# jgiovatto/srsLTE

Measured on AMD Instinct MI355X. Metric: turbo decoded Mbit/s (LTE 20 MHz, K=6144, 8 half-iterations) incl. OFDM demod of the same subframes, higher is better.
Workload: dtype int16

## Files before the change

srslte_amd/csrc/turbo_kernels.hip:

```cpp
#include <type_traits>

#include "hip_common.h"
#include "turbo_arith.h"
#include "turbo_device.h"
#include "turbo_extract.h"
#include "turbo_layout.h"

namespace phyhip {
namespace turbo {

template <class AR>
__device__ __forceinline__ void beta_step(s2 (&o)[8], s2 x, s2 y)
{
  auto adds = [](s2 a, s2 b) { return AR::add_raw(a, b); };
  s2   xy   = AR::add(x, y);
  s2 n0 = vmax(adds(o[4], xy), o[0]);
  s2 n1 = vmax(o[4], adds(o[0], xy));
  s2 n2 = vmax(adds(o[5], y), adds(o[1], x));
  s2 n3 = vmax(adds(o[5], x), adds(o[1], y));
  s2 n4 = vmax(adds(o[6], x), adds(o[2], y));
  s2 n5 = vmax(adds(o[6], y), adds(o[2], x));
  s2 n6 = vmax(o[7], adds(o[3], xy));
  s2 n7 = vmax(adds(o[7], xy), o[3]);
  o[0] = AR::clean(n0);
  o[1] = AR::clean(n1);
  o[2] = AR::clean(n2);
  o[3] = AR::clean(n3);
  o[4] = AR::clean(n4);
  o[5] = AR::clean(n5);
  o[6] = AR::clean(n6);
  o[7] = AR::clean(n7);
}

template <class AR, bool WITH_LLR>
__device__ __forceinline__ s2 alpha_step(s2 (&o)[8], const s2 (&b)[8], s2 x, s2 y)
{
  auto adds = [](s2 a, s2 b) { return AR::add_raw(a, b); };
  s2   xy   = AR::add(x, y);
  s2 m_b[8], nw[8];
  m_b[0] = o[0];
  m_b[1] = adds(o[3], y);
  m_b[2] = adds(o[4], y);
  m_b[3] = o[7];
  m_b[4] = o[1];
  m_b[5] = adds(o[2], y);
  m_b[6] = adds(o[5], y);
  m_b[7] = o[6];
  nw[0] = adds(o[1], xy);
  nw[1] = adds(o[2], x);
  nw[2] = adds(o[5], x);
  nw[3] = adds(o[6], xy);
  nw[4] = adds(o[0], xy);
  nw[5] = adds(o[3], x);
  nw[6] = adds(o[4], x);
  nw[7] = adds(o[7], xy);
  s2 out = splat(0);
  if (WITH_LLR) {
    s2 m0 = adds(b[0], m_b[0]);
    s2 m1 = adds(b[0], nw[0]);
#pragma unroll
    for (int i = 1; i < 8; i++) {
      m0 = vmax(m0, adds(b[i], m_b[i]));
      m1 = vmax(m1, adds(b[i], nw[i]));
    }
    out = AR::llr(AR::clean(m1), AR::clean(m0));
  }
#pragma unroll
  for (int i = 0; i < 8; i++) {
    o[i] = AR::clean(vmax(m_b[i], nw[i]));
  }
  return out;
}

__device__ __forceinline__ void keep_ops(uint4 (&Bl)[8][2][64], uint32_t s, int lane, const s2 (&xs)[8], const s2 (&ys)[8])
{
  Bl[2 * s][0][lane]     = make_uint4(to_u(xs[0]), to_u(xs[1]), to_u(xs[2]), to_u(xs[3]));
  Bl[2 * s][1][lane]     = make_uint4(to_u(xs[4]), to_u(xs[5]), to_u(xs[6]), to_u(xs[7]));
  Bl[2 * s + 1][0][lane] = make_uint4(to_u(ys[0]), to_u(ys[1]), to_u(ys[2]), to_u(ys[3]));
  Bl[2 * s + 1][1][lane] = make_uint4(to_u(ys[4]), to_u(ys[5]), to_u(ys[6]), to_u(ys[7]));
}
__device__ __forceinline__ void kept_ops(const uint4 (&Bl)[8][2][64], uint32_t s, int lane, s2 (&xs)[8], s2 (&ys)[8])
{
  const uint4 x0 = Bl[2 * s][0][lane], x1 = Bl[2 * s][1][lane], y0 = Bl[2 * s + 1][0][lane], y1 = Bl[2 * s + 1][1][lane];
  xs[0] = from_u(x0.x), xs[1] = from_u(x0.y), xs[2] = from_u(x0.z), xs[3] = from_u(x0.w);
  xs[4] = from_u(x1.x), xs[5] = from_u(x1.y), xs[6] = from_u(x1.z), xs[7] = from_u(x1.w);
  ys[0] = from_u(y0.x), ys[1] = from_u(y0.y), ys[2] = from_u(y0.z), ys[3] = from_u(y0.w);
  ys[4] = from_u(y1.x), ys[5] = from_u(y1.y), ys[6] = from_u(y1.z), ys[7] = from_u(y1.w);
}

__device__ __forceinline__ uint32_t norm_mask(bool on)
{
  uint32_t m = __builtin_amdgcn_readfirstlane(on ? ~0u : 0u);
  asm("" : "+s"(m));
  return m;
}

template <bool WHOLE, int POS>
struct FwdBody {
  static constexpr bool value = WHOLE;
  static constexpr int  pos   = POS;
};


template <int LPC, class AR, bool ES, int CKS>
__device__ __forceinline__ void tdec_win_unit(const WinParams& p, const uint32_t wb, const int lane, uint4 (&Bl)[8][2][64],
                                              uint32_t (&Tr)[512])
{
  const uint32_t crc_poly = ES ? p.crc_poly : 0u;
  const CbDesc*  desc     = ES ? p.desc : nullptr;
  constexpr int  NB  = 2 * LPC;
  constexpr int  CPW = 64 / LPC;
  constexpr bool NT  = !ES && !AR::kIs8;
  static_assert(CKS == 8 || CKS == 16, "check-points every 8 or every 16 steps");
  static_assert(CKS == 8 || !AR::kIs8, "the 16-step form's whole-block bodies use Ar16's masked normalisation");
  using ARW = std::conditional_t<CKS == 16, AR, Ar16>;
  const int     pl   = lane % LPC;
  const uint32_t xbase = xch_group_base<LPC>(lane);
  const int     cb_raw = (int)wb * CPW + lane / LPC;
  const bool    live = cb_raw < p.n_cb;
  const int     cb   = live ? cb_raw : p.n_cb - 1;
  const uint32_t K       = p.K;
  const uint32_t long_sb = K / NB;
  const uint32_t nblk    = (long_sb + 7) >> 3;
  const uint32_t AW      = nblk * LPC * 8;

  const uint32_t AWG = AW * CPW;
  uint32_t* ws  = p.ws + (size_t)wb * p.ws_stride * CPW;
  uint32_t* S   = ws;
  uint32_t* P0  = ws + AWG;
  uint32_t* P1  = ws + 2 * AWG;
  uint32_t* A1  = ws + 3 * AWG;
  uint32_t* D   = ws + 4 * AWG;
  uint32_t* A2  = ws + 5 * AWG;
  uint32_t* CK  = ws + 6 * AWG;
  short*    TL  = reinterpret_cast<short*>(CK + (size_t)(nblk + 1) * 64 * 8) + 16 * (lane / LPC);

  if (p.n_begin == 0) {
    const bool fast = !desc && !p.in_is8 && !p.sb_layout && (long_sb & 3u) == 0 && ((reinterpret_cast<uintptr_t>(p.input) | (2u * p.in_stride)) & 7u) == 0;
    if (fast) {
      const int first = (int)wb * CPW;
      extract_input_natural16<LPC, AR>(p.input + (size_t)first * p.in_stride, p.in_stride, p.n_cb - first, K, long_sb, nblk, lane,
                                       S, P0, P1, TL - 16 * (lane / LPC), reinterpret_cast<uint2*>(&Bl[0][0][0]));
    } else if (!p.in_is8 && p.sb_layout &&
               __all(((reinterpret_cast<uintptr_t>(p.input) + 2 * (desc ? (size_t)desc[cb].in_off : (size_t)cb * p.in_stride)) & 15u) == 0)) {
      const short* in = p.input + (desc ? (size_t)desc[cb].in_off : (size_t)cb * p.in_stride);
      extract_input_sb16<LPC, AR>(in, K, long_sb >> 3, lane, pl, S, P0, P1, TL, Tr);
      if (long_sb & 7u) {
        extract_input<LPC, AR>(in, 1, K, long_sb, nblk, lane, pl, S, P0, P1, TL, long_sb >> 3, false);
      }
    } else if (p.in_is8) {
      const signed char* in = reinterpret_cast<const signed char*>(p.input) + (desc ? (size_t)desc[cb].in_off : (size_t)cb * p.in_stride);
      extract_input<LPC, AR>(in, p.sb_layout, K, long_sb, nblk, lane, pl, S, P0, P1, TL);
    } else {
      const short* in = p.input + (desc ? (size_t)desc[cb].in_off : (size_t)cb * p.in_stride);
      extract_input<LPC, AR>(in, p.sb_layout, K, long_sb, nblk, lane, pl, S, P0, P1, TL);
    }
  }
  const uint32_t wrap_row = (AR::kIs8 && (K & 31u)) ? long_sb - 1 : 0xffffffffu;
  __syncthreads();

  uint8_t*       out       = p.output + (desc ? (size_t)desc[cb].out_off : (size_t)cb * p.out_stride);
  const uint32_t out_bytes = desc ? desc[cb].out_bytes : K / 8;
  uint32_t m_own_v = ~0u, m_row_v = ~0u;
  auto     set_masks = [&](bool dead) {
    const unsigned long long dm = __ballot(dead);
    const int                og = AR::kIs8 ? ((8 * (lane & 7)) / LPC) * LPC : ((4 * (lane & 15)) / LPC) * LPC;
    m_own_v                     = dead ? 0u : ~0u;
    m_row_v                     = ((dm >> og) & 1ull) ? 0u : ~0u;
  };
  if (ES) {
    set_masks(!live);
  }
  auto m_own = [&]() -> uint32_t { return ES ? m_own_v : ~0u; };
  auto m_row = [&]() -> uint32_t { return ES ? m_row_v : ~0u; };
  const bool bit_rows = !ES && p.final_run && !p.dec_llr && p.n_end > p.n_begin;
  auto decide = [&](bool write, bool final_try) -> uint32_t {
    short*         o16   = (p.dec_llr && live && write) ? p.dec_llr + (size_t)cb * K : nullptr;
    const bool     whole = (long_sb & 7) == 0;
    const uint32_t bps   = long_sb >> 3;
    const uint32_t poly  = crc_poly & 0xffffffu;
    uint32_t       c0 = 0, c1 = 0;
    const uint32_t sbs  = nblk + 1;
    uint8_t*       sbuf = reinterpret_cast<uint8_t*>(&Bl[0][0][0]) + (size_t)(lane / LPC) * NB * sbs;
    static_assert(sizeof(Bl) >= 64 / LPC * 2 * LPC * (6144 / (2 * LPC) / 8 + 2), "byte image does not fit");
    if (!whole) {
      sbuf[(2 * pl) * sbs + nblk]     = 0;
      sbuf[(2 * pl + 1) * sbs + nblk] = 0;
    }
    uint4* img = &Bl[0][0][0] + (whole ? 0u : (CPW * NB * sbs + 15u) / 16u);
    if (bit_rows) {
      for (uint32_t k = lane; k < long_sb; k += 64) {
        img[k] = ws_load16<NT>(D + (size_t)k * 4);
      }
      __syncthreads();
    }
    {
      const bool wide = whole && ((bps & 3) == 0) && ((reinterpret_cast<uintptr_t>(out) & 3) == 0) && out_bytes == K / 8;
      uint32_t   w0 = 0, w1 = 0;
      uint32_t   t[8], tn[8];
      if (!bit_rows) {
        issue_rows_raw<AR::kIs8, NT>(D, 0, lane, t);
      }
      for (uint32_t b = 0; b < nblk; b++) {
        if (!bit_rows && b + 1 < nblk) {
          issue_rows_raw<AR::kIs8, NT>(D, (b + 1) & m_row(), lane, tn);
        }
        uint32_t r[8];
        if (bit_rows) {
#pragma unroll
          for (int j = 0; j < 8; j++) {
            const uint32_t k = b * 8 + j < long_sb ? b * 8 + j : long_sb - 1;
            const uint4    m = img[k];
            r[j] = (uint32_t)(((((uint64_t)m.y << 32) | m.x) >> lane) & 1u) | ((uint32_t)(((((uint64_t)m.w << 32) | m.z) >> lane) & 1u) << 16);
          }
        } else {
          rows_to_lane_v<AR::kIs8>(Tr, lane, t, r);
        }
        uint32_t b0 = 0, b1 = 0;
#pragma unroll
        for (int j = 0; j < 8; j++) {
          if (b * 8 + j < long_sb) {
            const s2       v  = from_u(r[j]);
            const uint32_t x0 = v.x > 0 ? 1u : 0u, x1 = v.y > 0 ? 1u : 0u;
            b0 |= (x0 << 7) >> j;
            b1 |= (x1 << 7) >> j;
            if (crc_poly) {
              c0 = ((c0 << 1) & 0xffffffu) ^ ((((c0 >> 23) ^ x0) & 1u) ? poly : 0u);
              c1 = ((c1 << 1) & 0xffffffu) ^ ((((c1 >> 23) ^ x1) & 1u) ? poly : 0u);
            }
            if (o16 && whole) {
              o16[(2 * pl) * long_sb + b * 8 + j]     = AR::out16(v.x);
              o16[(2 * pl + 1) * long_sb + b * 8 + j] = AR::out16(v.y);
            }
          }
        }
        if (!whole) {
          sbuf[(2 * pl) * sbs + b]     = (uint8_t)b0;
          sbuf[(2 * pl + 1) * sbs + b] = (uint8_t)b1;
        }
        if (whole && write && live) {
          if (wide) {
            w0 |= b0 << (8 * (b & 3));
            w1 |= b1 << (8 * (b & 3));
            if ((b & 3) == 3) {
              *reinterpret_cast<uint32_t*>(out + (2 * pl) * bps + (b & ~3u))     = w0;
              *reinterpret_cast<uint32_t*>(out + (2 * pl + 1) * bps + (b & ~3u)) = w1;
              w0 = w1 = 0;
            }
          } else {
            if ((2 * pl) * bps + b < out_bytes) {
              out[(2 * pl) * bps + b] = (uint8_t)b0;
            }
            if ((2 * pl + 1) * bps + b < out_bytes) {
              out[(2 * pl + 1) * bps + b] = (uint8_t)b1;
            }
          }
        }
        if (!bit_rows) {
#pragma unroll
          for (int j = 0; j < 8; j++) {
            t[j] = tn[j];
          }
        }
      }
    }
    uint32_t crc = 0;
    if (crc_poly) {
      auto mulmod = [&](uint32_t a, uint32_t m) {
        uint32_t r = 0;
#pragma unroll 4
        for (int i = 23; i >= 0; i--) {
          r = ((r << 1) & 0xffffffu) ^ (((r >> 23) & 1u) ? poly : 0u);
          r ^= ((m >> i) & 1u) ? a : 0u;
        }
        return r;
      };
      crc = mulmod(c0, p.crc_mult[2 * pl]) ^ mulmod(c1, p.crc_mult[2 * pl + 1]);
#pragma unroll
      for (int off = LPC / 2; off > 0; off >>= 1) {
        crc ^= __shfl_xor(crc, off, LPC);
      }
    }
    __syncthreads();
    if (!whole && write && (!crc_poly || crc == 0 || final_try)) {
      const uint32_t nbytes = K / 8;
      const uint32_t lim    = out_bytes < nbytes ? out_bytes : nbytes;
      const bool     al     = (reinterpret_cast<uintptr_t>(out) & 3) == 0;
      for (uint32_t w = pl; w * 4 < nbytes; w += LPC) {
        uint32_t d = (w * 32) / long_sb, k = w * 32 - d * long_sb;
        uint32_t word = 0;
#pragma unroll
        for (int t = 0; t < 4; t++) {
          if (w * 4 + t < nbytes) {
            const uint8_t* q = sbuf + d * sbs + (k >> 3);
            uint32_t       v = ((((uint32_t)q[0] << 8) | q[1]) >> (8 - (k & 7))) & 0xffu;
            if (k + 8 > long_sb && d + 1 < (uint32_t)NB) {
              v |= (uint32_t)sbuf[(d + 1) * sbs] >> (long_sb - k);
            }
            word |= v << (8 * t);
          }
          k += 8;
          if (k >= long_sb) {
            k -= long_sb;
            d++;
          }
        }
        if (live) {
          if (al && w * 4 + 3 < lim) {
            *reinterpret_cast<uint32_t*>(out + 4 * w) = word;
          } else {
#pragma unroll
            for (int t = 0; t < 4; t++) {
              if (w * 4 + t < lim) {
                out[w * 4 + t] = (uint8_t)(word >> (8 * t));
              }
            }
          }
        }
      }
      if (o16) {
        const short* sd = reinterpret_cast<const short*>(D);
        for (uint32_t nn = pl; nn < K; nn += LPC) {
          const uint32_t d = nn / long_sb, k = nn % long_sb;
          const uint32_t e = (k * 64 + (lane / LPC) * LPC + (d >> 1)) * 2 + (d & 1);
          o16[nn] = AR::kIs8 ? (short)reinterpret_cast<const signed char*>(D)[e] : sd[e];
        }
      }
    }
    __syncthreads();
    return crc;
  };
  bool     done = false;
  uint32_t noi  = 0;

  for (uint32_t n = p.n_begin; n < p.n_end; n++) {
    const bool      dec1    = !(n & 1);
    const bool      has_app = dec1 && n > 0;
    const uint32_t* Y       = dec1 ? P0 : P1;
    const short*    xt      = dec1 ? TL : TL + 6;
    const short*    yt      = dec1 ? TL + 3 : TL + 9;

    struct Ops {
      uint32_t x[8], y[8], a[8];
    };
    constexpr std::integral_constant<bool, NT>    kStream{};
    constexpr std::integral_constant<bool, false> kReuse{};
    const uint32_t* X = dec1 ? S : A2;
    auto issue = [&](auto nt, uint32_t b, Ops& q, bool ok = true) {
      if constexpr (CKS == 16) {
        static_assert(!ES, "the early-stop masks differ between blocked and row arrays");
        const bool oka = ok && has_app;
        uint32_t   bb = ok ? b : 0u, ba = oka ? b : 0u;
        int        ln = ok ? lane : 0, la = oka ? lane : 0;
        asm volatile("" : "+v"(ln), "+v"(la));
        issue_rows_raw<AR::kIs8, nt.value>(X, bb, ln, q.x);
        issue_rows_raw<AR::kIs8, nt.value>(Y, bb, ln, q.y);
        issue_rows_raw<AR::kIs8, nt.value>(A1, ba, la, q.a);
      } else {
        if (dec1) {
          load_block_raw<AR::kIs8, NT>(S, (b & m_own()) * 64 + lane, q.x);
        } else {
          issue_rows_raw<AR::kIs8, NT>(A2, b & m_row(), lane, q.x);
        }
        load_block_raw<AR::kIs8, NT>(Y, (b & m_own()) * 64 + lane, q.y);
        if (has_app) {
          issue_rows_raw<AR::kIs8, NT>(A1, b & m_row(), lane, q.a);
        }
      }
    };
    auto prep = [&](const Ops& q, s2(&xs)[8], s2(&ys)[8], s2(&ap)[8]) {
      uint32_t xr[8], ar[8], yr[8];
      if (dec1) {
        block_values<AR::kIs8>(q.x, xr);
      } else {
        rows_to_lane_v<AR::kIs8>(Tr, lane, q.x, xr);
      }
      if (has_app) {
        rows_to_lane_v<AR::kIs8>(Tr, lane, q.a, ar);
      }
      block_values<AR::kIs8>(q.y, yr);
#pragma unroll
      for (int j = 0; j < 8; j++) {
        xs[j] = from_u(xr[j]);
        ys[j] = from_u(yr[j]);
        ap[j] = splat(0);
        if (has_app) {
          ap[j] = from_u(ar[j]);
          xs[j] = AR::add(ap[j], xs[j]);
        }
      }
    };
    auto taken = [&](const Ops& q) {
      asm volatile("" ::"v"(q.x[0]), "v"(q.x[1]), "v"(q.x[2]), "v"(q.x[3]), "v"(q.x[4]), "v"(q.x[5]), "v"(q.x[6]), "v"(q.x[7]));
      asm volatile("" ::"v"(q.y[0]), "v"(q.y[1]), "v"(q.y[2]), "v"(q.y[3]), "v"(q.y[4]), "v"(q.y[5]), "v"(q.y[6]), "v"(q.y[7]));
      if (has_app || CKS == 16) {
        asm volatile("" ::"v"(q.a[0]), "v"(q.a[1]), "v"(q.a[2]), "v"(q.a[3]), "v"(q.a[4]), "v"(q.a[5]), "v"(q.a[6]), "v"(q.a[7]));
      }
    };
    Ops cur, nxt, nx2, nx3;

    s2 fw[8];
#pragma unroll
    for (int i = 0; i < 8; i++) {
      fw[i] = splat(-AR::kInf);
    }
    {
      const uint32_t w0 = long_sb - TD_WIN_OVERLAP;
      const uint32_t bl = nblk - 1;
      issue(kStream, w0 >> 3, cur);
      for (uint32_t b = w0 >> 3; b <= bl; b++) {
        issue(kStream, b < bl ? b + 1 : TD_WIN_OVERLAP / 8 - 1, nxt);
        s2 xs[8], ys[8], ap[8];
        prep(cur, xs, ys, ap);
        if (b + 4 > bl) {
          keep_ops(Bl, b + 3 - bl, lane, xs, ys);
        }
#pragma unroll
        for (int j = 0; j < 8; j++) {
          uint32_t k = b * 8 + j;
          if (k >= w0 && k < long_sb) {
            alpha_step<AR, false>(fw, fw, xs[j], ys[j]);
            uint32_t kk = k - w0;
            if (AR::norm_at(kk)) {
              AR::normalize(fw);
            }
          }
        }
        cur = nxt;
      }
    }
#pragma unroll
    for (int i = 0; i < 8; i++) {
      uint32_t u   = to_u(fw[i]);
      uint32_t prv = __shfl_up(u, 1, LPC);
      uint32_t lo  = (pl == 0) ? (uint32_t)(uint16_t)(short)(i ? -AR::kInf : 0) : (prv >> 16);
      uint32_t hi  = u & 0xffffu;
      fw[i]        = from_u(lo | (hi << 16));
    }

    s2 o[8];
#pragma unroll
    for (int i = 0; i < 8; i++) {
      o[i] = splat(-AR::kInf);
    }
    for (int b = TD_WIN_OVERLAP / 8 - 1; b >= 0; b--) {
      if (b > 0) {
        issue(kStream, b - 1, nxt);
      }
      s2 xs[8], ys[8], ap[8];
      prep(cur, xs, ys, ap);
#pragma unroll
      for (int j = 7; j >= 0; j--) {
        beta_step<AR>(o, xs[j], ys[j]);
        uint32_t k = b * 8 + j;
        if (AR::norm_at(k)) {
          AR::normalize(o);
        }
      }
      cur = nxt;
    }
    {
      short tr[8];
      tail_trellis<AR>(xt, yt, tr);
#pragma unroll
      for (int i = 0; i < 8; i++) {
        uint32_t u   = to_u(o[i]);
        uint32_t nbr = __shfl_down(u, 1, LPC);
        uint32_t lo  = u >> 16;
        uint32_t hi  = (pl == LPC - 1) ? (uint32_t)(uint16_t)tr[i] : (nbr & 0xffffu);
        o[i]         = from_u(lo | (hi << 16));
      }
      uint32_t ck[8];
#pragma unroll
      for (int i = 0; i < 8; i++) {
        ck[i] = to_u(o[i]);
      }
      store_block_v<AR::kIs8>(CK, (nblk & m_own()) * 64 + lane, ck);
    }
    if constexpr (CKS == 16) {
      const int top = (int)nblk - 5;
      auto      block = [&](int b, const Ops& c, Ops& tgt) {
        s2 xs[8], ys[8], ap[8];
        if (b > top) {
          kept_ops(Bl, (uint32_t)(b < (int)nblk ? b : (int)nblk - 1) + 4 - nblk, lane, xs, ys);
        } else {
          taken(c);
          prep(c, xs, ys, ap);
        }
        issue(kStream, b - 3, tgt, b >= 3 && b - 3 <= top);
        if (b < (int)nblk) {
#pragma unroll
          for (int j = 7; j >= 0; j--) {
            uint32_t k = b * 8 + j;
            if (k < long_sb) {
              beta_step<AR>(o, xs[j], ys[j]);
              if (j == 0 && b > 0 && !(b & 1)) {
                uint32_t ck[8];
#pragma unroll
                for (int i = 0; i < 8; i++) {
                  ck[i] = to_u(o[i]);
                }
                store_block_v<AR::kIs8>(CK, ((uint32_t)b & m_own()) * 64 + lane, ck);
              }
              if (AR::norm_at(k)) {
                AR::normalize(o);
              }
            }
          }
        }
      };
      auto whole_block = [&](auto nt, auto ck_store, auto bottom, int b, const Ops& c, Ops& tgt) {
        s2 xs[8], ys[8], ap[8];
        taken(c);
        prep(c, xs, ys, ap);
        issue(nt, b - 3, tgt, b >= 3);
#pragma unroll
        for (int j = 7; j >= 0; j--) {
          beta_step<AR>(o, xs[j], ys[j]);
          if constexpr (ck_store.value) {
            if (j == 0) {
              uint32_t ck[8];
#pragma unroll
              for (int i = 0; i < 8; i++) {
                ck[i] = to_u(o[i]);
              }
              store_block_v<AR::kIs8>(CK, ((uint32_t)b & m_own()) * 64 + lane, ck);
            }
          }
          if (bottom.value && j == 0) {
            AR::normalize_if(o, norm_mask(b != 0));
          } else if (AR::norm_in_block(j)) {
            AR::normalize(o);
          }
        }
      };
      constexpr std::integral_constant<bool, true>  kStore{}, kBottom{};
      constexpr std::integral_constant<bool, false> kNoStore{}, kInner{};
      int b = ((int)nblk - 1) | 3;
#pragma nounroll
      for (; b > top; b -= 4) {
        block(b, nx3, cur);
        block(b - 1, nx2, nx3);
        block(b - 2, nxt, nx2);
        block(b - 3, cur, nxt);
      }
      const int b_reuse = p.reuse_blocks ? (int)p.reuse_blocks + 6 : 3;
#pragma nounroll
      for (; b >= b_reuse; b -= 4) {
        whole_block(kStream, kNoStore, kInner, b, nx3, cur);
        whole_block(kStream, kStore, kInner, b - 1, nx2, nx3);
        whole_block(kStream, kNoStore, kInner, b - 2, nxt, nx2);
        whole_block(kStream, kStore, kBottom, b - 3, cur, nxt);
      }
#pragma nounroll
      for (; b >= 3; b -= 4) {
        whole_block(kReuse, kNoStore, kInner, b, nx3, cur);
        whole_block(kReuse, kStore, kInner, b - 1, nx2, nx3);
        whole_block(kReuse, kNoStore, kInner, b - 2, nxt, nx2);
        whole_block(kReuse, kStore, kBottom, b - 3, cur, nxt);
      }
    } else {
      for (int b = (int)nblk - 1; b >= 0; b--) {
        const bool ahead = b + 3 <= (int)nblk;
        if (b > 1 && ahead) {
          issue(kStream, b - 2, nx2);
        }
        s2 xs[8], ys[8], ap[8];
        if (b + 4 >= (int)nblk) {
          kept_ops(Bl, (uint32_t)b + 4 - nblk, lane, xs, ys);
        } else {
          prep(cur, xs, ys, ap);
        }
#pragma unroll
        for (int j = 7; j >= 0; j--) {
          uint32_t k = b * 8 + j;
          if (k < long_sb) {
            beta_step<AR>(o, xs[j], ys[j]);
            if (j == 0 && b > 0 && (CKS == 8 || !(b & 1))) {
              uint32_t ck[8];
#pragma unroll
              for (int i = 0; i < 8; i++) {
                ck[i] = to_u(o[i]);
              }
              store_block_v<AR::kIs8>(CK, ((uint32_t)b & m_own()) * 64 + lane, ck);
            }
            if (AR::norm_at(k)) {
              AR::normalize(o);
            }
          }
        }
        if (b > 0 && ahead) {
          cur = nxt;
          nxt = nx2;
        }
      }
    }
    __syncthreads();

#pragma unroll
    for (int i = 0; i < 8; i++) {
      o[i] = fw[i];
    }

    const uint32_t* lut = dec1 ? p.deint : p.inter;
    uint32_t*       dst = dec1 ? A2 : A1;
    const bool fuse = dec1 && n >= 2;
    uint32_t sub_x = dec1 ? 0u : ~0u;
    asm volatile("" : "+s"(sub_x));
    const bool last = (n + 1 == p.n_end) || crc_poly;
    const bool sign_rows = bit_rows && n + 1 == p.n_end;

    constexpr FwdBody<false, -1> kGeneral{};
    constexpr FwdBody<true, 0>   kWhole0{};
    constexpr FwdBody<true, 1>   kWhole1{};
    constexpr FwdBody<true, 2>   kWhole2{};
    constexpr FwdBody<true, 3>   kWhole3{};
    auto rederive_start = [&](int len, const uint32_t(&ckv)[8], s2(&st)[8]) {
#pragma unroll
      for (int i = 0; i < 8; i++) {
        st[i] = from_u(ckv[i]);
      }
      const int top = CKS == 16 ? (len - 1) & 7 : len - 1;
      Bl[top][0][lane] = make_uint4(ckv[0], ckv[1], ckv[2], ckv[3]);
      Bl[top][1][lane] = make_uint4(ckv[4], ckv[5], ckv[6], ckv[7]);
    };
    auto rederive_rest = [&](auto whole, uint32_t b, int len, const s2(&xs)[8], const s2(&ys)[8], s2(&st)[8]) {
#pragma unroll
      for (int j = 6; j >= 0; j--) {
        if (whole.value || j <= len - 2) {
          uint32_t idx = b * 8 + j + 2;
          if constexpr (whole.pos == 3) {
            if (j == 6) {
              ARW::normalize_if(st, norm_mask(idx != long_sb));
            } else if (AR::norm_in_block(j + 2)) {
              AR::normalize(st);
            }
          } else if (whole.value ? AR::norm_in_block(j + 2) : (idx != long_sb && AR::norm_at(idx))) {
            AR::normalize(st);
          }
          beta_step<AR>(st, xs[j + 1], ys[j + 1]);
          Bl[j][0][lane] = make_uint4(to_u(st[0]), to_u(st[1]), to_u(st[2]), to_u(st[3]));
          Bl[j][1][lane] = make_uint4(to_u(st[4]), to_u(st[5]), to_u(st[6]), to_u(st[7]));
        }
      }
    };
    auto emit = [&](auto whole, uint32_t b, int len, const s2(&xs)[8], const s2(&ys)[8], const s2(&ap)[8], const uint32_t(&tr)[8], auto&& ck_taken) {
      uint32_t outv[8], rawv[8];
#pragma unroll
      for (int j = 0; j < 8; j++) {
        outv[j] = 0;
        rawv[j] = 0;
        if (whole.value || j < len) {
          const uint4 b0 = Bl[j][0][lane], b1 = Bl[j][1][lane];
          const s2    B[8] = {from_u(b0.x), from_u(b0.y), from_u(b0.z), from_u(b0.w),
                              from_u(b1.x), from_u(b1.y), from_u(b1.z), from_u(b1.w)};
          s2       llr = alpha_step<AR, true>(o, B, xs[j], ys[j]);
          uint32_t k   = b * 8 + j;
          if constexpr (whole.pos == 0) {
            if (j == 0) {
              ARW::normalize_if(o, norm_mask(k != 0));
            } else if (AR::norm_in_block(j)) {
              AR::normalize(o);
            }
          } else if (whole.value ? AR::norm_in_block(j) : AR::norm_at(k)) {
            AR::normalize(o);
          }
          s2 proc = llr;
          if constexpr (!AR::kIs8) {
            proc = AR::ex_sub(llr, from_u(to_u(ap[j]) | (to_u(xs[j]) & sub_x)), false);
          } else if (fuse) {
            proc = AR::ex_sub(llr, ap[j], k == wrap_row);
          } else if (!dec1) {
            proc = AR::ex_sub(llr, xs[j], xch_row(tr[j]) == wrap_row);
          }
          outv[j] = to_u(proc);
          rawv[j] = to_u(llr);
        }
      }
      if constexpr (CKS == 16) {
        asm volatile("" ::"v"(tr[0]), "v"(tr[1]), "v"(tr[2]), "v"(tr[3]), "v"(tr[4]), "v"(tr[5]), "v"(tr[6]), "v"(tr[7]));
        ck_taken();
      }
      if (!sign_rows) {
        if constexpr (whole.value) {
          uint32_t xv[8];
#pragma unroll
          for (int j = 0; j < 8; j++) {
            xv[j] = permute_pair(outv[j], tr[j], xbase);
          }
#pragma unroll
          for (int j = 0; j < 8; j++) {
            store_xch_row<AR::kIs8>(dst, tr[j], m_own(), lane, xv[j]);
          }
        } else {
#pragma unroll
          for (int j = 0; j < 8; j++) {
            if (j < len) {
              store_xch_row<AR::kIs8>(dst, tr[j], m_own(), lane, permute_pair(outv[j], tr[j], xbase));
            }
          }
        }
      }
      if (last) {
#pragma unroll
        for (int j = 0; j < 8; j++) {
          if (whole.value || j < len) {
            if (sign_rows) {
              const s2       v  = from_u(dec1 ? rawv[j] : permute_pair(rawv[j], tr[j], xbase));
              const uint64_t mx = __ballot(v.x > 0), my = __ballot(v.y > 0);
              if (lane == 0) {
                *reinterpret_cast<uint4*>(D + (size_t)(dec1 ? b * 8 + j : xch_row(tr[j]) & m_own()) * 4) =
                    make_uint4((uint32_t)mx, (uint32_t)(mx >> 32), (uint32_t)my, (uint32_t)(my >> 32));
              }
            } else if (dec1) {
              store_row<AR::kIs8>(D, (b * 8 + j) & m_own(), lane, rawv[j]);
            } else {
              store_xch_row<AR::kIs8>(D, tr[j], m_own(), lane, permute_pair(rawv[j], tr[j], xbase));
            }
          }
        }
      }
    };

    if constexpr (CKS == 8) {
      uint32_t ck[8], tr[8], ckn[8], trn[8];
      load_block_raw<AR::kIs8, NT>(CK, (1u & m_own()) * 64 + lane, ck);
      load_lut(lut, pl, tr);
      if (nblk > 1) {
        issue(kStream, 1, nxt);
      }
      for (uint32_t b = 0; b < nblk; b++) {
        const int len = (long_sb - b * 8) < 8 ? (int)(long_sb - b * 8) : 8;
        s2        xs[8], ys[8], ap[8];
        if (b + 2 < nblk) {
          issue(kStream, b + 2, nx2);
        }
        if (b + 1 < nblk) {
          load_block_raw<AR::kIs8, NT>(CK, ((b + 2) & m_own()) * 64 + lane, ckn);
          load_lut(lut, (b + 1) * LPC + pl, trn);
        }
        prep(cur, xs, ys, ap);
        uint32_t ckv[8];
        block_values<AR::kIs8>(ck, ckv);
        s2 st[8];
        rederive_start(len, ckv, st);
        rederive_rest(kGeneral, b, len, xs, ys, st);
        emit(kGeneral, b, len, xs, ys, ap, tr, [] {});
        cur = nxt;
        nxt = nx2;
#pragma unroll
        for (int i = 0; i < 8; i++) {
          ck[i] = ckn[i];
          tr[i] = trn[i];
        }
      }
    } else {
      Ops&     q0 = cur;
      Ops&     q1 = nxt;
      Ops&     q2 = nx2;
      Ops&     q3 = nx3;
      uint32_t ck[8], tr[8];
      load_block_raw<AR::kIs8, NT>(CK, ((nblk < 2 ? nblk : 2u) & m_own()) * 64 + lane, ck);
      issue(kStream, 1, q1, nblk > 1);
      asm volatile("" ::"v"(ck[0]), "v"(ck[1]), "v"(ck[2]), "v"(ck[3]), "v"(ck[4]), "v"(ck[5]), "v"(ck[6]), "v"(ck[7]));
      taken(q1);
      issue(kStream, 2, q2, nblk > 2);
      auto block = [&](auto whole, auto even, uint32_t b, const Ops& c, const Ops& held, Ops& tgt) {
        const int rem = (int)long_sb - (int)b * 8;
        const int len = whole.value ? 8 : rem < 0 ? 0 : rem < 8 ? rem : 8;
        s2         xs[8], ys[8], ap[8], st[8];
        uint32_t   ckv[8];
        auto       ck_taken = [&] { asm volatile("" ::"v"(ck[0]), "v"(ck[1]), "v"(ck[2]), "v"(ck[3]), "v"(ck[4]), "v"(ck[5]), "v"(ck[6]), "v"(ck[7])); };
        ck_taken();
        block_values<AR::kIs8>(ck, ckv);
        load_lut(lut, (whole.value || b < nblk ? b : nblk - 1) * LPC + pl, tr);
        taken(c);
        if constexpr (even.value) {
          taken(held);
          issue(kStream, b + 3, tgt, b + 3 < nblk);
        } else {
          prep(c, xs, ys, ap);
          rederive_start(len, ckv, st);
          const uint32_t bn = b + 3 < nblk ? b + 3 : nblk;
          load_block_raw<AR::kIs8, NT>(CK, (bn & m_own()) * 64 + lane, ck);
          issue(kStream, b + 3, tgt, b + 3 < nblk);
        }
        {
          if constexpr (even.value) {
            const bool paired = whole.value || b + 1 < nblk;
            s2        x1[8], y1[8], a1[8];
            if (paired) {
              prep(held, x1, y1, a1);
            }
            prep(c, xs, ys, ap);
            if (paired) {
              const int len1 = whole.value ? 8 : (long_sb - (b + 1) * 8) < 8 ? (int)(long_sb - (b + 1) * 8) : 8;
#pragma unroll
              for (int i = 0; i < 8; i++) {
                st[i] = from_u(ckv[i]);
              }
#pragma unroll
              for (int j = 7; j >= 0; j--) {
                if (whole.value || j < len1) {
                  uint32_t idx = (b + 1) * 8 + j + 1;
                  if constexpr (whole.pos == 2) {
                    if (j == 7) {
                      AR::normalize_if(st, norm_mask(idx != long_sb));
                    } else if (AR::norm_in_block(j + 1)) {
                      AR::normalize(st);
                    }
                  } else if (whole.value ? AR::norm_in_block(j + 1) : (idx != long_sb && AR::norm_at(idx))) {
                    AR::normalize(st);
                  }
                  beta_step<AR>(st, x1[j], y1[j]);
                }
              }
#pragma unroll
              for (int i = 0; i < 8; i++) {
                ckv[i] = to_u(st[i]);
              }
            }
            rederive_start(len, ckv, st);
          }
          rederive_rest(whole, b, len, xs, ys, st);
          emit(whole, b, len, xs, ys, ap, tr, ck_taken);
        }
      };
      constexpr std::integral_constant<bool, true>  kEven{};
      constexpr std::integral_constant<bool, false> kOdd{};
      uint32_t       b  = 0;
      const uint32_t wl = (long_sb & 31u) ? 5u : 4u;
#pragma nounroll
      for (int trip = 0; trip < 2; trip++) {
        const uint32_t gend = trip == 0 ? (wl <= nblk ? 0u : 4u) : nblk;
#pragma nounroll
        for (; b < gend; b += 4) {
          block(kGeneral, kEven, b, q0, q1, q3);
          block(kGeneral, kOdd, b + 1, q1, q2, q0);
          block(kGeneral, kEven, b + 2, q2, q3, q1);
          block(kGeneral, kOdd, b + 3, q3, q0, q2);
        }
#pragma nounroll
        for (; b + wl <= nblk; b += 4) {
          block(kWhole0, kEven, b, q0, q1, q3);
          block(kWhole1, kOdd, b + 1, q1, q2, q0);
          block(kWhole2, kEven, b + 2, q2, q3, q1);
          block(kWhole3, kOdd, b + 3, q3, q0, q2);
        }
      }
    }
    __syncthreads();
    if (crc_poly) {
      const bool     last_try = n + 1 == p.n_end;
      const bool     wr       = !done;
      const uint32_t crc      = decide(wr, last_try);
      if (!done) {
        noi++;
        done = crc == 0;
      }
      set_masks(done || !live);
      __syncthreads();
      if (__all(done || !live) || last_try) {
        break;
      }
    }
  }

  if (!crc_poly) {
    decide(true, true);
  } else if (p.noi && live && pl == 0) {
    p.noi[cb_raw]    = (int)noi;
    p.crc_ok[cb_raw] = done ? 1 : 0;
  }
}

template <class AR, bool ES>
constexpr int win_ck_spacing = (!AR::kIs8 && !ES) ? 16 : 8;

template <int LPC, class AR, bool ES, int CKS = win_ck_spacing<AR, ES>>
__global__ __launch_bounds__(64) __attribute__((amdgpu_waves_per_eu(2, 2))) void tdec_win_kernel(const WinParams p)
{
  __shared__ uint4    Bl[8][2][64];
  __shared__ uint32_t Tr[512];
  tdec_win_unit<LPC, AR, ES, CKS>(p, blockIdx.x, threadIdx.x, Bl, Tr);
}


template <bool ES>
static hipError_t launch_win_es(int nb, bool arith8, const WinParams& p, hipStream_t stream)
{
  const int lpc = nb / 2;
  dim3      grid(ceil_div(p.n_cb, 64 / lpc));
  if (!arith8 && nb == 16) {
    hipLaunchKernelGGL((tdec_win_kernel<8, Ar16, ES>), grid, dim3(64), 0, stream, p);
  } else if (!arith8 && nb == 8) {
    hipLaunchKernelGGL((tdec_win_kernel<4, Ar16, ES>), grid, dim3(64), 0, stream, p);
  } else if (arith8 && nb == 16) {
    hipLaunchKernelGGL((tdec_win_kernel<8, Ar8, ES>), grid, dim3(64), 0, stream, p);
  } else if (arith8 && nb == 32) {
    hipLaunchKernelGGL((tdec_win_kernel<16, Ar8, ES>), grid, dim3(64), 0, stream, p);
  } else {
    return hipErrorInvalidValue;
  }
  return hipGetLastError();
}

hipError_t launch_win(int nb, bool arith8, const WinParams& p, hipStream_t stream)
{
  return (p.crc_poly || p.desc) ? launch_win_es<true>(nb, arith8, p, stream) : launch_win_es<false>(nb, arith8, p, stream);
}

uint32_t win_elem_index(int nb, uint32_t k, uint32_t d)
{
  return nb == 32 ? elem_index<16>(k, d) : (nb == 16 ? elem_index<8>(k, d) : elem_index<4>(k, d));
}

}
}
```

Before: 43550.

## Carry backward-recursion tail blocks in registers into forward pass start

```diff
diff --git a/srslte_amd/csrc/turbo_kernels.hip b/srslte_amd/csrc/turbo_kernels.hip
--- a/srslte_amd/csrc/turbo_kernels.hip
+++ b/srslte_amd/csrc/turbo_kernels.hip
@@ -398,6 +398,8 @@
       }
     };
     Ops cur, nxt, nx2, nx3;
+    const bool turned = CKS == 16 && nblk >= 8;
+    uint32_t   ck2[8];
 
     s2 fw[8];
 #pragma unroll
@@ -509,11 +511,11 @@
           }
         }
       };
-      auto whole_block = [&](auto nt, auto ck_store, auto bottom, int b, const Ops& c, Ops& tgt) {
+      auto whole_block = [&](auto nt, auto ck_store, int b, const Ops& c, Ops& tgt) {
         s2 xs[8], ys[8], ap[8];
         taken(c);
         prep(c, xs, ys, ap);
-        issue(nt, b - 3, tgt, b >= 3);
+        issue(nt, b - 3, tgt);
 #pragma unroll
         for (int j = 7; j >= 0; j--) {
           beta_step<AR>(o, xs[j], ys[j]);
@@ -527,15 +529,33 @@
               store_block_v<AR::kIs8>(CK, ((uint32_t)b & m_own()) * 64 + lane, ck);
             }
           }
-          if (bottom.value && j == 0) {
-            AR::normalize_if(o, norm_mask(b != 0));
+          if (AR::norm_in_block(j)) {
+            AR::normalize(o);
+          }
+        }
+      };
+      auto turn_block = [&](auto first, const Ops& c) {
+        s2 xs[8], ys[8], ap[8];
+        taken(c);
+        prep(c, xs, ys, ap);
+        if constexpr (first.value) {
+          issue(kStream, 0, cur);
+        }
+#pragma unroll
+        for (int j = 7; j >= 0; j--) {
+          beta_step<AR>(o, xs[j], ys[j]);
+          if (!first.value && j == 0) {
+#pragma unroll
+            for (int i = 0; i < 8; i++) {
+              ck2[i] = to_u(o[i]);
+            }
           } else if (AR::norm_in_block(j)) {
             AR::normalize(o);
           }
         }
       };
-      constexpr std::integral_constant<bool, true>  kStore{}, kBottom{};
-      constexpr std::integral_constant<bool, false> kNoStore{}, kInner{};
+      constexpr std::integral_constant<bool, true>  kStore{};
+      constexpr std::integral_constant<bool, false> kNoStore{};
       int b = ((int)nblk - 1) | 3;
 #pragma nounroll
       for (; b > top; b -= 4) {
@@ -544,20 +564,24 @@
         block(b - 2, nxt, nx2);
         block(b - 3, cur, nxt);
       }
-      const int b_reuse = p.reuse_blocks ? (int)p.reuse_blocks + 6 : 3;
+      const int b_reuse = p.reuse_blocks ? (int)p.reuse_blocks + 6 : 7;
 #pragma nounroll
       for (; b >= b_reuse; b -= 4) {
-        whole_block(kStream, kNoStore, kInner, b, nx3, cur);
-        whole_block(kStream, kStore, kInner, b - 1, nx2, nx3);
-        whole_block(kStream, kNoStore, kInner, b - 2, nxt, nx2);
-        whole_block(kStream, kStore, kBottom, b - 3, cur, nxt);
+        whole_block(kStream, kNoStore, b, nx3, cur);
+        whole_block(kStream, kStore, b - 1, nx2, nx3);
+        whole_block(kStream, kNoStore, b - 2, nxt, nx2);
+        whole_block(kStream, kStore, b - 3, cur, nxt);
       }
 #pragma nounroll
-      for (; b >= 3; b -= 4) {
-        whole_block(kReuse, kNoStore, kInner, b, nx3, cur);
-        whole_block(kReuse, kStore, kInner, b - 1, nx2, nx3);
-        whole_block(kReuse, kNoStore, kInner, b - 2, nxt, nx2);
-        whole_block(kReuse, kStore, kBottom, b - 3, cur, nxt);
+      for (; b >= 7; b -= 4) {
+        whole_block(kReuse, kNoStore, b, nx3, cur);
+        whole_block(kReuse, kStore, b - 1, nx2, nx3);
+        whole_block(kReuse, kNoStore, b - 2, nxt, nx2);
+        whole_block(kReuse, kStore, b - 3, cur, nxt);
+      }
+      if (turned) {
+        turn_block(std::true_type{}, nx3);
+        turn_block(std::false_type{}, nx2);
       }
     } else {
       for (int b = (int)nblk - 1; b >= 0; b--) {
@@ -759,12 +783,19 @@
       Ops&     q1 = nxt;
       Ops&     q2 = nx2;
       Ops&     q3 = nx3;
-      uint32_t ck[8], tr[8];
-      load_block_raw<AR::kIs8, NT>(CK, ((nblk < 2 ? nblk : 2u) & m_own()) * 64 + lane, ck);
-      issue(kStream, 1, q1, nblk > 1);
-      asm volatile("" ::"v"(ck[0]), "v"(ck[1]), "v"(ck[2]), "v"(ck[3]), "v"(ck[4]), "v"(ck[5]), "v"(ck[6]), "v"(ck[7]));
-      taken(q1);
-      issue(kStream, 2, q2, nblk > 2);
+      uint32_t(&ck)[8] = ck2;
+      uint32_t tr[8];
+      if (!turned) {
+        load_block_raw<AR::kIs8, NT>(CK, ((nblk < 2 ? nblk : 2u) & m_own()) * 64 + lane, ck);
+        issue(kStream, 1, q1, nblk > 1);
+        asm volatile("" ::"v"(ck[0]), "v"(ck[1]), "v"(ck[2]), "v"(ck[3]), "v"(ck[4]), "v"(ck[5]), "v"(ck[6]), "v"(ck[7]));
+        taken(q1);
+        issue(kStream, 2, q2, nblk > 2);
+      } else {
+        taken(q1);
+        taken(q2);
+        taken(q0);
+      }
       auto block = [&](auto whole, auto even, uint32_t b, const Ops& c, const Ops& held, Ops& tgt) {
         const int rem = (int)long_sb - (int)b * 8;
         const int len = whole.value ? 8 : rem < 0 ? 0 : rem < 8 ? rem : 8;
```

Result: faster. 44080 (median of 6 runs) (+1.2%).
